# jeffpeterson/hypermerge

Measured on AMD Instinct MI355X. Metric: merged changes/sec (1M docs×8 actors) at 1/2/4/8 GPUs + % HBM roofline, higher is better.
Workload: dtype u32; 1 GPU; C4: 1000000 docs/GPU x 8 actors x 64 changes/doc, map LWW sets; docs_per_gpu=1000000, changes_per_gpu=64000000, ops_per_gpu=96000538, parallelism=doc-shard1

## Files before the change

### hypermerge_amd/csrc/merge_kernels.hip

```cpp
#include <hip/hip_runtime.h>
#include <stdint.h>
#include "../../include/hypermerge_amd.h"
#include "merge_kernels.h"
#include "wave.h"

#ifndef HM_ABLATE
#define HM_ABLATE 0
#endif
#ifndef HM_STAMPS
#define HM_STAMPS 0
#endif
#define HM_NSTAMP 20
#ifndef HM_WAVES_PER_EU_OPL4
#define HM_WAVES_PER_EU_OPL4 3
#endif
#ifndef HM_WAVES_PER_EU_LIST3
#define HM_WAVES_PER_EU_LIST3 3
#endif
#ifndef HM_PRIO_PUSH
#define HM_PRIO_PUSH 2
#endif
#ifndef HM_PRIO_IO
#define HM_PRIO_IO 1
#endif
// ... 6 lines not shown
#ifndef HM_PRIO_K2
#define HM_PRIO_K2 2
#endif
#ifndef HM_PRIO_K1
#define HM_PRIO_K1 3
#endif
#ifndef HM_ASYNC_MAX_OPL
#define HM_ASYNC_MAX_OPL 2
#endif
#ifndef HM_ASYNC_STORES
#define HM_ASYNC_STORES 10
#endif
#ifndef HM_ASYNC_CHECK
#define HM_ASYNC_CHECK 0
#endif
#ifndef HM_WAVES_PER_EU
#define HM_WAVES_PER_EU 5
#endif
#ifndef HM_WAVES_PER_EU_WIDE
#define HM_WAVES_PER_EU_WIDE 4
#endif
#define WAVE 64
#define NA_MAX 8
#define NDEP_MAX 1024
typedef unsigned long long u64;
#if defined(__HIP_DEVICE_COMPILE__)
#define LDS __attribute__((address_space(3)))
#else
#define LDS
#endif

namespace hm {

__device__ __forceinline__ u64 readlane64(u64 v, int l) {
    const uint32_t lo = __builtin_amdgcn_readlane((int)(uint32_t)v, l);
    const uint32_t hi = __builtin_amdgcn_readlane((int)(uint32_t)(v >> 32), l);
    return ((u64)hi << 32) | lo;
}
__device__ __forceinline__ uint32_t shfl32(uint32_t v, int src) {
    return (uint32_t)__builtin_amdgcn_ds_bpermute(src << 2, (int)v);
}
__device__ __forceinline__ u64 shfl64(u64 v, int src) {
    return ((u64)shfl32((uint32_t)(v >> 32), src) << 32) | shfl32((uint32_t)v, src);
}
__device__ __forceinline__ u64 wave_or64(u64 v) {
    for (int o = 1; o < WAVE; o <<= 1) v |= shfl64(v, (int)(threadIdx.x ^ o));
    return v;
}
__device__ __forceinline__ uint32_t wave_excl_scan(uint32_t v, uint32_t *total) {
    uint32_t x = v;
    x += (uint32_t)__builtin_amdgcn_update_dpp(0, (int)x, DPP_ROW_SHR(1), 0xF, 0xF, false);
    x += (uint32_t)__builtin_amdgcn_update_dpp(0, (int)x, DPP_ROW_SHR(2), 0xF, 0xF, false);
    x += (uint32_t)__builtin_amdgcn_update_dpp(0, (int)x, DPP_ROW_SHR(4), 0xF, 0xF, false);
    x += (uint32_t)__builtin_amdgcn_update_dpp(0, (int)x, DPP_ROW_SHR(8), 0xF, 0xF, false);
    x += (uint32_t)__builtin_amdgcn_update_dpp(0, (int)x, DPP_ROW_BCAST15, 0xA, 0xF, false);
    x += (uint32_t)__builtin_amdgcn_update_dpp(0, (int)x, DPP_ROW_BCAST31, 0xC, 0xF, false);
    *total = (uint32_t)__builtin_amdgcn_readlane((int)x, WAVE - 1);
    return x - v;
}
__device__ __forceinline__ uint32_t wave_max(uint32_t v) {
    uint32_t x = v, y;
    y = (uint32_t)__builtin_amdgcn_update_dpp(0, (int)x, DPP_ROW_SHR(1), 0xF, 0xF, false); x = x > y ? x : y;
    y = (uint32_t)__builtin_amdgcn_update_dpp(0, (int)x, DPP_ROW_SHR(2), 0xF, 0xF, false); x = x > y ? x : y;
    y = (uint32_t)__builtin_amdgcn_update_dpp(0, (int)x, DPP_ROW_SHR(4), 0xF, 0xF, false); x = x > y ? x : y;
    y = (uint32_t)__builtin_amdgcn_update_dpp(0, (int)x, DPP_ROW_SHR(8), 0xF, 0xF, false); x = x > y ? x : y;
    y = (uint32_t)__builtin_amdgcn_update_dpp(0, (int)x, DPP_ROW_BCAST15, 0xA, 0xF, false); x = x > y ? x : y;
    y = (uint32_t)__builtin_amdgcn_update_dpp(0, (int)x, DPP_ROW_BCAST31, 0xC, 0xF, false); x = x > y ? x : y;
    return (uint32_t)__builtin_amdgcn_readlane((int)x, WAVE - 1);
}
__device__ __forceinline__ uint32_t bytesum64(u64 x) {
    return __builtin_amdgcn_sad_u8((uint32_t)x, 0u, __builtin_amdgcn_sad_u8((uint32_t)(x >> 32), 0u, 0u));
}
__device__ __forceinline__ uint32_t prev_lane(uint32_t v) {
    return (uint32_t)__builtin_amdgcn_update_dpp(0, (int)v, DPP_WAVE_SHR1, 0xF, 0xF, false);
}
__device__ __forceinline__ uint32_t fresh_lane() {
    uint32_t l;
    asm volatile("v_mov_b32 %0, %1" : "=v"(l) : "v"((uint32_t)threadIdx.x));
    return l;
}
template <bool FRESH> __device__ __forceinline__ uint32_t lane_id() {
    if constexpr (FRESH) return fresh_lane();
    else return threadIdx.x;
}
template <int OPL, bool LISTS, int CLS> struct Diet { static constexpr bool on = OPL <= 2 && !LISTS && CLS != 1; };
__device__ __forceinline__ void wave_sync() {
    __builtin_amdgcn_fence(__ATOMIC_SEQ_CST, "wavefront");
    __builtin_amdgcn_wave_barrier();
}

__device__ __forceinline__ u64 err_key(uint32_t h, uint32_t op_plus1, uint32_t arr, uint32_t code) {
    return ((u64)h << 40) | ((u64)(op_plus1 & 0xFFFF) << 24) | ((u64)(arr & 0xFFFF) << 8) | code;
}

struct SmallLds {
    LDS u64 *anc, *chain, *segor, *errkey, *cov;
    LDS u64 *opval;
    LDS u64 *survpk;
    LDS int64_t *survsum;
    LDS uint32_t *first, *base, *bclock, *headv, *objslot, *segcnt, *survcnt, *regoff, *regobj, *insmin;
    LDS uint32_t *flags, *deps, *depinfo;
    LDS uint8_t *seglist;
    LDS uint16_t *survp;
    LDS uint32_t *opro;
    LDS uint32_t *opmeta;
    LDS uint32_t *opelem;
    LDS int32_t *hist_of;
    LDS uint16_t *survop, *opbase;
    LDS uint16_t *oppar;
    LDS uint8_t *h2a, *chactor, *objtype;
    LDS uint16_t *opchg;
    LDS uint32_t *nins, *pcount, *nodekey, *tour0, *listbase;
    LDS uint16_t *poff;
    LDS uint16_t *nodeop, *nodepi, *regnode, *plist, *fc, *ns, *listid;
    LDS u64 *stamps;
};
#define PAR_HEAD 0xFFFFu
template <bool LISTS> struct Stride {
    static constexpr uint32_t reg = LISTS ? 1 : 4;
    static constexpr uint32_t seg = LISTS ? 1 : 2;
    static constexpr uint32_t op = LISTS ? 1 : 2;
};

template <int CLS> struct SizeClass;
template <> struct SizeClass<0> { static constexpr uint32_t NR = 32, NO = 16, ND = 128; };
template <> struct SizeClass<1> { static constexpr uint32_t NR = 256, NO = 64, ND = 512; };
template <> struct SizeClass<2> { static constexpr uint32_t NR = 128, NO = 32, ND = 256; };

template <typename L_t, typename P>
__host__ __device__ inline size_t small_carve(P base, uint32_t NOp, uint32_t NR, uint32_t NO, uint32_t ND,
                                              bool lists, bool counters, L_t *L) {
    size_t o = 0;
#define TAKE(f, T, cnt) do { L->f = (decltype(L->f))(base + o); o = (o + (size_t)(cnt) * sizeof(T) + 15) & ~(size_t)15; } while (0)
    TAKE(anc, u64, 64);          TAKE(chain, u64, NA_MAX);     TAKE(opval, u64, NOp);
    TAKE(errkey, u64, 1);        TAKE(base, uint32_t, NA_MAX * 3);
    if (lists) {
        TAKE(survcnt, uint32_t, NR); TAKE(regoff, uint32_t, NR);   TAKE(regobj, uint32_t, NR);
        TAKE(insmin, uint32_t, NR);  TAKE(flags, uint32_t, 2);
        TAKE(opmeta, uint32_t, NOp); TAKE(opro, uint32_t, NOp);
    } else {
        TAKE(survcnt, uint32_t, 4 * NR);                           TAKE(flags, uint32_t, 2);
        L->regoff = L->survcnt + 1; L->insmin = L->survcnt + 2;    L->regobj = L->survcnt + 3;
        TAKE(opro, uint32_t, 2 * NOp);
        L->opmeta = L->opro + 1;
    }
    TAKE(survop, uint16_t, NOp); TAKE(chactor, uint8_t, 64);   TAKE(objtype, uint8_t, NO);
    if (lists) {
        TAKE(opelem, uint32_t, NOp);
        L->nodekey = L->opelem;
        TAKE(nins, uint32_t, 1);
    }
    TAKE(stamps, u64, HM_STAMPS ? HM_NSTAMP + 1 : 0);
    const size_t dead_at = o;
    TAKE(hist_of, int32_t, 64);  TAKE(cov, u64, 1);            TAKE(opbase, uint16_t, 64);
    TAKE(oppar, uint16_t, lists ? NOp : 0);
    TAKE(h2a, uint8_t, 64);      TAKE(opchg, uint16_t, NOp);
    const size_t k1_at = o;
    TAKE(first, uint32_t, NA_MAX * 64);
    TAKE(deps, uint32_t, ND > NOp ? ND : NOp);
    TAKE(depinfo, uint32_t, ND);
    const size_t k1_end = o;
    o = k1_at;
    if (lists) { TAKE(segor, u64, NR);  TAKE(survpk, u64, NR); }
    else { TAKE(segor, u64, 2 * NR);    L->survpk = L->segor + 1; }
    TAKE(segcnt, uint32_t, NR);
    TAKE(objslot, uint32_t, NO);
    if (o < k1_end) o = k1_end;
    L->seglist = (decltype(L->seglist))L->first; L->survp = (decltype(L->survp))L->first;
    if (lists) {
        const uint32_t NP = NR + NO, NE = 2 * (NOp + NO);
        size_t q = dead_at;
#define TAKEK(f, T, cnt) do { L->f = (decltype(L->f))(base + q); q = (q + (size_t)(cnt) * sizeof(T) + 15) & ~(size_t)15; } while (0)
        TAKEK(tour0, uint32_t, NE);     TAKEK(pcount, uint32_t, NP);  TAKEK(listbase, uint32_t, NO + 1);
        TAKEK(poff, uint16_t, NP + 1);  TAKEK(survp, uint16_t, NOp);
        TAKEK(nodeop, uint16_t, NOp);   TAKEK(nodepi, uint16_t, NOp); TAKEK(regnode, uint16_t, NR);
        TAKEK(plist, uint16_t, NOp);    TAKEK(fc, uint16_t, NP);      TAKEK(ns, uint16_t, NOp);
        TAKEK(listid, uint16_t, NO);    TAKEK(seglist, uint8_t, NOp);
#undef TAKEK
        if (q > o) o = q;
    }
    TAKE(survsum, int64_t, counters ? NOp : 0);
#undef TAKE
    L->bclock = L->base + NA_MAX;
    L->headv = L->base + 2 * NA_MAX;
    return o;
}

template <typename T> struct Id { typedef T type; };
template <typename T> __device__ __forceinline__ T lds_or(LDS T *p, typename Id<T>::type v) { return __atomic_fetch_or(p, v, __ATOMIC_RELAXED); }
template <typename T> __device__ __forceinline__ T lds_min(LDS T *p, typename Id<T>::type v) { return __atomic_fetch_min(p, v, __ATOMIC_RELAXED); }
template <typename T> __device__ __forceinline__ T lds_max(LDS T *p, typename Id<T>::type v) { return __atomic_fetch_max(p, v, __ATOMIC_RELAXED); }
template <typename T> __device__ __forceinline__ T lds_add(LDS T *p, typename Id<T>::type v) { return __atomic_fetch_add(p, v, __ATOMIC_RELAXED); }

#if HM_STAMPS
__device__ unsigned long long hm_stamp_acc[HM_NSTAMP];
__device__ __forceinline__ u64 stamp_now() {
    u64 t;
    __builtin_amdgcn_sched_barrier(0);
    asm volatile("s_memtime %0\n\ts_waitcnt lgkmcnt(0)" : "=s"(t) :: "memory");
    __builtin_amdgcn_sched_barrier(0);
    return t;
}
#define STAMP(L_, i) do { const u64 t_ = stamp_now(); if (threadIdx.x == 0) { (L_).stamps[i] += t_ - (L_).stamps[HM_NSTAMP]; (L_).stamps[HM_NSTAMP] = t_; } } while (0)
#elif defined(HM_MARKS)
#define STAMP(L_, i) asm volatile(";HMMARK " #i)
#else
#define STAMP(L_, i) do { } while (0)
#endif

enum : uint32_t { FL_UNSUPPORTED = 1u };
enum Outcome { OUT_OK = 0, OUT_ERROR = 1, OUT_UNSUPPORTED = 2, OUT_INVALID = 3 };

__device__ __forceinline__ void need_set(uint32_t &lo, uint32_t &hi, uint32_t a, uint32_t v) {
    const uint32_t sh = (a & 3) * 8;
    const uint32_t w = a < 4 ? lo : hi;
    const uint32_t cur = (w >> sh) & 0xFF;
    const uint32_t nw = v > cur ? ((w & ~(0xFFu << sh)) | (v << sh)) : w;
    lo = a < 4 ? nw : lo;
    hi = a < 4 ? hi : nw;
}


__device__ __forceinline__ uint32_t fidx(uint32_t a, uint32_t s) { return (s & 63) * NA_MAX + (a & (NA_MAX - 1)); }
__device__ __forceinline__ void clear_first(LDS uint32_t *first, uint32_t lane) {
    static_assert(NA_MAX * 64 == 2 * WAVE * 4, "first-table size");
    LDS uint4 *f4 = (LDS uint4 *)first;
    const uint4 ones = make_uint4(~0u, ~0u, ~0u, ~0u);
    f4[lane] = ones;
    f4[lane + WAVE] = ones;
}

__device__ __forceinline__ uint32_t tie_order(uint32_t pc) { return (pc & 1) ? (0x10000u - pc) : (0x20000u + pc); }


template <int OPL>
__device__ __forceinline__ void rga_order(const SmallLds &L, uint32_t R, uint32_t O,
                                          const uint32_t (&oreg)[OPL], const uint32_t (&oobj)[OPL],
                                          const uint32_t (&opar)[OPL], const uint32_t (&oact)[OPL],
                                          const uint32_t (&oelem)[OPL], const uint32_t (&oarr)[OPL],
// ... 327 lines not shown
        if (lane < n) f(lane);
        if constexpr (CAP > WAVE) { if (lane + WAVE < n) f(lane + WAVE); }
    } else {
        for (uint32_t i = lane; i < n; i += WAVE) f(i);
    }
}
template <int OPL, bool LISTS, bool DIET, typename C>
__device__ __forceinline__ void stage_rows(const SmallParams &p, const SmallLds &L, const hm_doc_row &doc, const Rows &r) {
    const uint32_t lane = lane_id<DIET>(), m = doc.n_ops;
    stage_op<LISTS>(L, lane, m, r.a0, r.b0);
    if (OPL > 1) stage_op<LISTS>(L, lane + WAVE, m, r.a1, r.b1);
    if (OPL > 2) stage_op<LISTS>(L, lane + 2 * WAVE, m, r.a2, r.b2);
    if (OPL > 3) stage_op<LISTS>(L, lane + 3 * WAVE, m, r.a3, r.b3);
    const uint32_t nd = doc.n_deps < C::ND ? doc.n_deps : C::ND;
    if (lane < nd) L.deps[lane] = pack_dep(r.d0);
    if (lane + WAVE < nd) L.deps[lane + WAVE] = pack_dep(r.d1);
    if constexpr (C::ND > 2 * WAVE)
        for (uint32_t i = lane + 2 * WAVE; i < nd; i += WAVE)
            L.deps[i] = pack_dep(*reinterpret_cast<const uint2 *>(p.deps + doc.dep_off + i));
}
__device__ __forceinline__ hm_change_row change_of(uint2 w0, uint2 w1, uint2 w2) {
    hm_change_row c;
    c.actor = (uint16_t)(w0.x & 0xFFFF); c.n_deps = (uint16_t)(w0.x >> 16); c.seq = w0.y;
    c.dep_off = w1.x; c.n_ops = w1.y; c.op_first = w2.x; c.content_id = w2.y;
    return c;
}
struct DocState {
    int32_t hist;
    uint32_t H, total;
    bool doc_lists;
    bool counters;
};

struct OpCheck { uint32_t err; bool surv, has_list, late; };
template <bool LISTS>
__device__ __forceinline__ OpCheck op_check(const SmallLds &L, int32_t ohv, uint32_t act, uint32_t obj, uint32_t reg,
                                            uint32_t par, uint32_t okey, uint32_t R, uint32_t O) {
    const bool asg = ohv >= 0 && act >= HM_INS && act <= HM_INC && reg < R;
    const uint32_t oi = obj < O ? obj : 0u, ri = reg < R ? reg : 0u;
    const uint32_t os = obj < O ? L.objslot[oi] : 0xFFFFFFFFu;
    const uint32_t pi = par < R ? par : 0u;
    uint32_t ot = 0, im = 0, ip = 0;
    if constexpr (LISTS) { ot = L.objtype[oi]; im = L.insmin[ri]; ip = L.insmin[pi]; }
    const u64 so = L.segor[Stride<LISTS>::seg * ri];
    const uint32_t h = ohv < 0 ? 0u : (uint32_t)ohv;
    const bool unknown = asg && (os == 0xFFFFFFFFu || os > okey);
    const bool known = asg && !unknown;
    if constexpr (!LISTS) {
        OpCheck r;
        r.has_list = false; r.late = false;
        r.surv = known && (act == HM_SET || act == HM_LINK) && !((so >> h) & 1);
        r.err = unknown ? (uint32_t)HM_ERR_UNKNOWN_OBJECT : 0u;
        return r;
    }
    const bool is_list = ot == HM_MAKE_LIST || ot == HM_MAKE_TEXT;
    const bool ins = known && act == HM_INS;
    const bool sl = known && (act == HM_SET || act == HM_LINK);
    OpCheck r;
    r.has_list = ins || (known && is_list);
    r.surv = sl && !((so >> h) & 1);
    r.late = ins && par != HM_HEAD && !(ip <= okey);
    uint32_t e = 0;
    if (sl && is_list && !(im <= okey)) e = HM_ERR_MISSING_ELEM;
    if (ins && im != okey + 1) e = HM_ERR_DUPLICATE_ELEM;
    if (unknown) e = HM_ERR_UNKNOWN_OBJECT;
    r.err = e;
    return r;
}

template <int OPL, bool LISTS, bool DIET, typename C>
__device__ __forceinline__ Outcome merge_doc_small(const SmallParams &p, const SmallLds &L, const hm_doc_row &doc,
                                                   const uint2 w0, const uint2 w1, const uint2 w2, DocState &st) {
    uint32_t lane = lane_id<DIET>();
    constexpr uint32_t RS = Stride<LISTS>::reg, SS = Stride<LISTS>::seg, OS = Stride<LISTS>::op;
    const uint32_t n = doc.n_changes, A = doc.n_actors, m = doc.n_ops, R = doc.n_regs, O = doc.n_objs;
    st.hist = -1; st.H = 0; st.total = 0; st.doc_lists = false; st.counters = false;

    if (HM_ABLATE & 8) return OUT_UNSUPPORTED;
    STAMP(L, 0);
    if (HM_PRIO_K1) __builtin_amdgcn_s_setprio(HM_PRIO_K1);
    const bool act = lane < n;
    const hm_change_row c = change_of(w0, w1, w2);
    clear_first(L.first, lane);
    if (lane < NA_MAX) { L.base[lane] = 0xFFFFFFFFu; L.bclock[lane] = 0; L.headv[lane] = 0; L.chain[lane] = 0; }
    if (lane == 0) { *L.errkey = ~0ull; L.flags[0] = 0; L.flags[1] = 0; *L.cov = 0; }
    const uint32_t dep_lo = doc.dep_off, ndep = doc.n_deps;
    wave_sync();
    const uint32_t actor = c.actor, seq = c.seq;
    const uint32_t my_dep0 = c.dep_off - dep_lo;
    const uint32_t op_end = c.op_first + c.n_ops, dep_end = c.dep_off + c.n_deps;
    const uint32_t prev_op = prev_lane(op_end), prev_dep = prev_lane(dep_end);
    bool bad = (n == 0 && (m || ndep)) ||
               (act && (c.op_first != (lane ? prev_op : doc.op_off) || c.dep_off != (lane ? prev_dep : dep_lo) ||
                        (lane == n - 1 && (op_end != doc.op_off + m || dep_end != dep_lo + ndep))));
    const bool rowok = act && !(actor >= A || seq == 0 || c.dep_off < dep_lo || my_dep0 + c.n_deps > ndep);
    bad |= act && !rowok;
    bad |= act && (c.op_first < doc.op_off || c.op_first - doc.op_off + c.n_ops > m);
    const uint32_t a8 = actor & (NA_MAX - 1);
    lds_min(&L.base[a8], rowok ? seq : 0xFFFFFFFFu);
    lds_max(&L.bclock[a8], rowok ? seq : 0u);
    L.chactor[lane] = (uint8_t)actor;
    L.opbase[lane] = (uint16_t)(c.op_first - doc.op_off);
    if (__ballot(bad)) return OUT_UNSUPPORTED;
    wave_sync();
    const uint32_t mybase = act ? L.base[a8] : 0;
    const uint32_t slot = seq - mybase;
    if (__ballot(act && slot >= 64)) return OUT_UNSUPPORTED;
    lds_min(&L.first[fidx(a8, (slot & 63))], act ? lane : 0xFFFFFFFFu);
    {
        const uint32_t o0 = c.op_first - doc.op_off;
        if (act) for (uint32_t j = 0; j < c.n_ops; j++) L.opchg[o0 + j] = (uint16_t)(lane | (a8 << 8));
    }
    wave_sync();

    STAMP(L, 1);
    if constexpr (DIET) lane = fresh_lane();
    if (HM_ABLATE & 16) return OUT_UNSUPPORTED;
    {
        bool bad_dep = false;
        for_rows<C::ND, LISTS>(lane, ndep, [&](uint32_t i) {
            const uint32_t pk = L.deps[i];
            const uint32_t a = pk >> 24, s = pk & 0xFFFFFF;
            bad_dep |= pk == 0xFFFFFFFFu || a >= A;
            const uint32_t ad = a & (NA_MAX - 1);
            const uint32_t b = L.base[ad];
            const bool inwin = b != 0xFFFFFFFFu && s >= b && s - b < 64;
            const uint32_t f = L.first[fidx(ad, ((s - b) & 63))];
            const uint32_t rel = s == 0 ? 0u : (inwin ? s - b + 1 : 0x7Fu);
            L.depinfo[i] = (inwin && f < 64 ? f : 0x7Fu) | (rel << 8) | (ad << 16);
        });
        if (__ballot(bad_dep)) return OUT_UNSUPPORTED;
    }
    const uint32_t first_me = act ? L.first[fidx(actor, slot)] : lane;
    const bool dup = act && first_me != lane;
    const uint32_t cid_first = shfl32(c.content_id, (int)(first_me & 63));
    u64 dmask = 0;
    uint32_t pred_arr = 0xFFu;
    bool ok = true;
    bool own_row = false;
    wave_sync();
    {
        const uint32_t maxd = wave_max(act ? (uint32_t)c.n_deps : 0u);
        for (uint32_t j0 = 0; j0 < maxd; j0 += 2) {
            uint32_t inf[2];
#pragma unroll
            for (int u = 0; u < 2; u++) {
                const bool live = act && j0 + u < c.n_deps;
                inf[u] = L.depinfo[live ? my_dep0 + j0 + u : 0u];
            }
#pragma unroll
            for (int u = 0; u < 2; u++) {
                const bool live = act && j0 + u < c.n_deps;
                const uint32_t a = (inf[u] >> 16) & (NA_MAX - 1), rel = (inf[u] >> 8) & 0x7F, f = inf[u] & 0x7F;
                own_row |= live && a == actor;
                const bool use = live && a != actor && rel != 0;
                ok = ok && !(use && (rel == 0x7F || f >= lane));
                dmask |= (use && rel != 0x7F && f < lane) ? (1ull << f) : 0ull;
            }
        }
        const uint32_t ps = seq - 1;
        const bool hp = act && ps != 0, inb = ps >= mybase;
        const uint32_t f = L.first[fidx(a8, ((ps - mybase) & 63))];
        ok = ok && !(hp && (!inb || f >= lane));
        const bool pv = hp && inb && f < lane;
        dmask |= pv ? (1ull << (f & 63)) : 0ull;
        pred_arr = pv ? f : pred_arr;
        ok = ok && !(dup && cid_first != c.content_id);
    }
    wave_sync();

    STAMP(L, 2);
    if constexpr (DIET) lane = fresh_lane();
    if (HM_ABLATE & 32) return OUT_UNSUPPORTED;
    int32_t hist = -1;
    uint32_t H = 0;
    bool identity = false;
    if (HM_PRIO_K1) __builtin_amdgcn_s_setprio(0);
    const bool queued_doc = __ballot(act && !ok) != 0;
    if (HM_PRIO_HIST && queued_doc) __builtin_amdgcn_s_setprio(HM_PRIO_HIST);
    if (!queued_doc) {
        const u64 appl = __ballot(act && !dup);
        if (act) hist = dup ? -2 : (int32_t)__popcll(appl & ((1ull << lane) - 1));
        H = (uint32_t)__popcll(appl);
        identity = __ballot(dup) == 0;
    } else if (__ballot(dup && cid_first != c.content_id) == 0) {
        u64 dall = 0;
        bool never = false;
        uint32_t pred_any = 0xFFu;
        {
            const uint32_t maxd = wave_max(act ? (uint32_t)c.n_deps : 0u);
            for (uint32_t j = 0; j < maxd; j++) {
                const bool live = act && j < c.n_deps;
                const uint32_t inf = L.depinfo[live ? my_dep0 + j : 0u];
                const uint32_t a = (inf >> 16) & (NA_MAX - 1), rel = (inf >> 8) & 0x7F, f = inf & 0x7F;
                const bool use = live && a != actor && rel != 0;
                never |= use && (rel == 0x7F || f == 0x7F);
                dall |= (use && rel != 0x7F && f != 0x7F) ? (1ull << f) : 0ull;
            }
            const uint32_t ps = seq - 1;
            const bool hp = act && ps != 0, inb = ps >= mybase;
            const uint32_t f = L.first[fidx(a8, ((ps - mybase) & 63))];
            never |= hp && (!inb || f >= 64);
            dall |= (hp && inb && f < 64) ? (1ull << f) : 0ull;
            pred_any = (hp && inb && f < 64) ? f : 0xFFu;
        }
        const u64 dupm = __ballot(dup), nodupm = __ballot(act && !dup);
        const u64 below = (1ull << lane) - 1;
        const uint32_t key = first_me & 63;
        u64 applied = 0, queue = 0;
        bool copy_applied = false;
        bool solved = false;
        {
            LDS uint32_t *tx = (LDS uint32_t *)L.hist_of;
            LDS uint32_t *tm = (LDS uint32_t *)L.anc;
            const uint32_t INF = 0xFFu;
            const bool has_dup = dupm != 0;
            const bool kl = act && !dup;
            uint32_t t = (!kl || never) ? INF : lane;
            const bool regdp = __ballot(act && __popcll(dall) > 4) == 0;
            uint32_t sl0 = lane, sl1 = lane, sl2 = lane, sl3 = lane;
            if (regdp) {
                u64 m = dall;
                sl0 = m ? (uint32_t)__builtin_ctzll(m) : lane; m &= m - 1;
                sl1 = m ? (uint32_t)__builtin_ctzll(m) : lane; m &= m - 1;
                sl2 = m ? (uint32_t)__builtin_ctzll(m) : lane; m &= m - 1;
                sl3 = m ? (uint32_t)__builtin_ctzll(m) : lane;
                for (uint32_t it = 0; it <= n; it++) {
                    const uint32_t x0 = shfl32(t, (int)sl0), x1 = shfl32(t, (int)sl1);
                    const uint32_t x2 = shfl32(t, (int)sl2), x3 = shfl32(t, (int)sl3);
                    uint32_t nt = t;
                    nt = nt > x0 ? nt : x0; nt = nt > x1 ? nt : x1; nt = nt > x2 ? nt : x2; nt = nt > x3 ? nt : x3;
                    nt = (kl && t != INF) ? nt : t;
                    const bool grew = nt != t;
                    t = nt;
                    if (__ballot(grew) == 0) break;
                }
            } else {
                for (uint32_t it = 0; it <= n; it++) {
                    tx[lane] = t;
                    wave_sync();
                    uint32_t nt = t;
                    if (kl && t != INF)
                        for (u64 m = dall; m; m &= m - 1) { const uint32_t x = tx[__builtin_ctzll(m)]; nt = nt > x ? nt : x; }
                    wave_sync();
                    const bool grew = nt != t;
                    t = nt;
                    if (__ballot(grew) == 0) break;
                }
            }
            STAMP(L, 13);
            tx[lane] = t;
            wave_sync();
            const uint32_t tk = act ? tx[key] : INF;
            wave_sync();
            uint32_t w = (!kl || t == INF) ? 0xFFFFFFFFu : ((t << 16) | ((t == lane ? 1u : 2u) << 8) | lane);
            bool conv = false;
            if (regdp) {
                const bool queued_copy = act && tk != INF && tk != key && lane < tk;
                const uint32_t nsl = (uint32_t)__popcll(dall);
                for (uint32_t it = 0; it <= n + 1; it++) {
                    const uint32_t y0 = shfl32(w, (int)sl0), y1 = shfl32(w, (int)sl1);
                    const uint32_t y2 = shfl32(w, (int)sl2), y3 = shfl32(w, (int)sl3);
                    uint32_t pc = 2;
                    auto fold = [&](uint32_t wd, uint32_t k) {
                        const uint32_t v = ((wd >> 8) & 0xFFu) + ((wd & 0xFFu) > lane ? 1u : 0u);
                        pc = (k < nsl && (wd >> 16) == tk && v > pc) ? v : pc;
                    };
                    fold(y0, 0); fold(y1, 1); fold(y2, 2); fold(y3, 3);
                    const uint32_t cand = queued_copy ? ((tk << 16) | ((pc > 0xFEu ? 0xFEu : pc) << 8) | lane) : 0xFFFFFFFFu;
                    uint32_t nw = w;
                    if (has_dup) {
                        tm[lane] = 0xFFFFFFFFu;
                        wave_sync();
                        if (cand != 0xFFFFFFFFu) lds_min(&tm[key], cand);
// ... 112 lines not shown
                if (seq - 1 != 0) { pred_arr = L.first[fidx(actor, (seq - 1 - mybase))]; dmask |= 1ull << pred_arr; }
            }
        }
    } else {
        uint32_t need_lo = 0, need_hi = 0;
        if (act) {
#pragma unroll 1
            for (uint32_t j = 0; j < c.n_deps; j++) {
                const uint32_t inf = L.depinfo[my_dep0 + j];
                const uint32_t a = (inf >> 16) & (NA_MAX - 1), rel = (inf >> 8) & 0x7F;
                need_set(need_lo, need_hi, a, (a != actor && rel != 0) ? rel : 0u);
            }
            const uint32_t ps = seq - 1;
            need_set(need_lo, need_hi, a8, ps != 0 ? (ps >= mybase ? ps - mybase + 1 : 0x7Fu) : 0u);
        }
        clear_first(L.first, lane);
        wave_sync();
        uint32_t crel_lo = 0, crel_hi = 0;
        u64 queued = 0;
        bool stop = false;
        for (uint32_t i = 0; i < n && !stop; i++) {
            queued |= 1ull << i;
            u64 above = 0;
            bool first_pass = true;
            for (;;) {
                bool progress = false;
                for (;;) {
                    const uint32_t x0 = ((crel_lo | 0x80808080u) - need_lo) & 0x80808080u;
                    const uint32_t x1 = ((crel_hi | 0x80808080u) - need_hi) & 0x80808080u;
                    u64 r = __ballot(act && x0 == 0x80808080u && x1 == 0x80808080u) & queued;
                    r &= first_pass ? (1ull << i) : above;
                    if (!r) break;
                    const uint32_t j = (uint32_t)__builtin_ctzll(r);
                    const uint32_t aj = (uint32_t)__builtin_amdgcn_readlane((int)actor, (int)j);
                    const uint32_t sj = (uint32_t)__builtin_amdgcn_readlane((int)slot, (int)j);
                    const uint32_t sh = (aj & 3) * 8;
                    const uint32_t cur = (((aj < 4) ? crel_lo : crel_hi) >> sh) & 0xFF;
                    queued &= ~(1ull << j);
                    progress = true;
                    above = (j >= 63) ? 0 : (~0ull << (j + 1));
                    if (sj + 1 <= cur) {
                        const uint32_t k = L.first[fidx(aj, sj)];
                        const uint32_t ck = (uint32_t)__builtin_amdgcn_readlane((int)c.content_id, (int)k);
                        const uint32_t cj = (uint32_t)__builtin_amdgcn_readlane((int)c.content_id, (int)j);
                        if (lane == j) hist = -2;
                        if (ck != cj) {
                            if (lane == 0) lds_min(L.errkey, err_key(H, 0, j, HM_ERR_INCONSISTENT_SEQ));
                            stop = true;
                            break;
                        }
                        if (first_pass) break;
                        continue;
                    }
                    if (aj < 4) crel_lo = (crel_lo & ~(0xFFu << sh)) | ((sj + 1) << sh);
                    else        crel_hi = (crel_hi & ~(0xFFu << sh)) | ((sj + 1) << sh);
                    if (lane == 0) L.first[fidx(aj, sj)] = j;
                    if (lane == j) hist = (int32_t)H;
                    H++;
                    if (first_pass) break;
                }
                if (stop || !progress) break;
                first_pass = false;
                above = ~0ull;
            }
        }
        wave_sync();
        dmask = 0; pred_arr = 0xFFu;
        if (act && hist >= 0) {
            for (uint32_t j = 0; j < c.n_deps; j++) {
                const uint32_t pk = L.deps[my_dep0 + j];
                const uint32_t a = pk >> 24, s = pk & 0xFFFFFF;
                if (a == actor || s == 0) continue;
                dmask |= 1ull << L.first[fidx(a, (s - L.base[a]))];
            }
            if (seq - 1 != 0) { pred_arr = L.first[fidx(actor, (seq - 1 - mybase))]; dmask |= 1ull << pred_arr; }
        }
    }

    if (HM_PRIO_HIST && queued_doc) __builtin_amdgcn_s_setprio(0);
    STAMP(L, 3);
    if constexpr (DIET) lane = fresh_lane();
    if (HM_ABLATE & 512) return OUT_UNSUPPORTED;
    if (act) L.hist_of[lane] = hist;
    if (act && hist >= 0) L.h2a[hist] = (uint8_t)lane;
    wave_sync();
    const bool hv = lane < H;
    uint32_t ai = lane, hactor = actor, hseq = seq, hpred = pred_arr;
    u64 dm_arr = dmask;
    if (!identity) {
        ai = hv ? L.h2a[lane] : 0;
        dm_arr = shfl64(dmask, (int)ai);
        hactor = shfl32(actor, (int)ai); hseq = shfl32(seq, (int)ai); hpred = shfl32(pred_arr, (int)ai);
    }
    u64 D = 0, Dnp = 0;
    if (identity) {
        D = hv ? dm_arr : 0ull;
        Dnp = hv && hpred != 0xFFu ? D & ~(1ull << hpred) : D;
    } else if (hv) {
        u64 x = dm_arr;
        while (x) {
            const uint32_t j = (uint32_t)__builtin_ctzll(x);
            x &= x - 1;
            const u64 bit = 1ull << (uint32_t)L.hist_of[j];
            D |= bit;
            if (j != hpred) Dnp |= bit;
        }
    }
    if (hv) { lds_or(L.cov, D); lds_or(&L.chain[hactor], 1ull << lane); }
    uint32_t alo = hv && lane < 32 ? 1u << lane : 0u, ahi = hv && lane >= 32 ? 1u << (lane - 32) : 0u;
    if (HM_ABLATE & 1024) return OUT_UNSUPPORTED;
    {
        if (HM_PRIO_PUSH) __builtin_amdgcn_s_setprio(HM_PRIO_PUSH);
        const uint32_t Hs = (uint32_t)__builtin_amdgcn_readfirstlane((int)H);
        const uint32_t Dlo = (uint32_t)D, Dhi = (uint32_t)(D >> 32);
        const uint32_t H1 = Hs < 32 ? Hs : 32;
#define PUSH_BC(v, k) ((uint32_t)__builtin_amdgcn_readlane((int)(v), (int)(k)))
#define PUSH_LO(k) alo |= PUSH_BC(alo, (k)) & (uint32_t)__builtin_amdgcn_sbfe((int)Dlo, (k), 1)
#define PUSH_HI(k) do { const uint32_t m_ = (uint32_t)__builtin_amdgcn_sbfe((int)Dhi, (k) - 32, 1);          \
                        const uint32_t bl_ = PUSH_BC(alo, (k)), bh_ = PUSH_BC(ahi, (k));                   \
                        alo |= bl_ & m_; ahi |= bh_ & m_; } while (0)
#pragma unroll
        for (int g = 0; g < 32; g += 8) {
            if ((uint32_t)g >= H1) break;
            PUSH_LO(g); PUSH_LO(g + 1); PUSH_LO(g + 2); PUSH_LO(g + 3);
            PUSH_LO(g + 4); PUSH_LO(g + 5); PUSH_LO(g + 6); PUSH_LO(g + 7);
        }
#pragma unroll
        for (int g = 32; g < 64; g += 8) {
            if ((uint32_t)g >= Hs) break;
            PUSH_HI(g); PUSH_HI(g + 1); PUSH_HI(g + 2); PUSH_HI(g + 3);
            PUSH_HI(g + 4); PUSH_HI(g + 5); PUSH_HI(g + 6); PUSH_HI(g + 7);
        }
#undef PUSH_LO
#undef PUSH_HI
#undef PUSH_BC
        if (HM_PRIO_PUSH) __builtin_amdgcn_s_setprio(0);
    }
    const u64 anc = hv ? ((((u64)ahi << 32) | alo) & ~(1ull << lane)) : 0ull;
    if (hv) L.anc[lane] = anc;
    wave_sync();
    STAMP(L, 4);
    if constexpr (DIET) lane = fresh_lane();
    if (HM_ABLATE & 64) return OUT_UNSUPPORTED;
    const u64 covered = *L.cov;
    bool suspect = false;
    if constexpr (LISTS) {
        if (hv && (Dnp & (Dnp - 1))) {
            u64 x = Dnp;
            while (x) {
                const uint32_t i2 = (uint32_t)__builtin_ctzll(x);
                x &= x - 1;
                if (L.anc[i2] & Dnp) suspect = true;
            }
        }
    } else {
        const u64 rest = Dnp & (Dnp - 1);
        const bool two = hv && rest != 0;
        if (__ballot(two)) {
            const u64 a1 = L.anc[two ? (uint32_t)__builtin_ctzll(rest) : 0u];
            u64 x = two ? rest & (rest - 1) : 0ull;
            suspect = two && (a1 & Dnp) != 0;
            if (__ballot(x != 0)) {
                while (x) {
                    const uint32_t i2 = (uint32_t)__builtin_ctzll(x);
                    x &= x - 1;
                    if (L.anc[i2] & Dnp) suspect = true;
                }
            }
        }
    }
    uint32_t h_own_row = own_row ? 1u : 0u, h_dep0 = my_dep0, h_nd = c.n_deps;
    if (!identity) {
        h_own_row = shfl32(h_own_row, (int)ai); h_dep0 = shfl32(my_dep0, (int)ai); h_nd = shfl32(c.n_deps, (int)ai);
    }
    suspect |= hv && h_own_row != 0;
    if (suspect) {
        const FoldView fv = {L.anc, L.chain, L.first, L.base, L.deps, L.hist_of};
        if (fold_differs(fv, h_dep0, h_nd, hactor, hseq)) lds_or(L.flags, FL_UNSUPPORTED);
    }
    if (hv && !((covered >> lane) & 1)) L.headv[hactor] = hseq;
    for_rows<C::NO, LISTS>(lane, O, [&](uint32_t i) {
        L.objslot[i] = i == 0 ? 0u : 0xFFFFFFFFu;
        if constexpr (LISTS) L.objtype[i] = i == 0 ? HM_MAKE_MAP : 0xFF;
    });
    for_rows<C::NR, LISTS>(lane, R, [&](uint32_t i) {
        if constexpr (LISTS) {
            L.segor[i] = 0; L.segcnt[i] = 0; L.survpk[i] = 0; L.insmin[i] = 0xFFFFFFFFu; L.regobj[i] = HM_NONE;
        } else {
            static_assert(Stride<false>::reg == 4 && Stride<false>::seg == 2, "row widths");
            *(LDS uint4 *)(L.survcnt + 4 * i) = make_uint4(0u, 0u, 0xFFFFFFFFu, HM_NONE);
            *(LDS uint4 *)(L.segor + 2 * i) = make_uint4(0u, 0u, 0u, 0u);
            L.segcnt[i] = 0;
        }
    });
    wave_sync();

    STAMP(L, 5);
    if constexpr (DIET) lane = fresh_lane();
    if (HM_PRIO_K2) __builtin_amdgcn_s_setprio(HM_PRIO_K2);
    if (HM_ABLATE & 2) return OUT_UNSUPPORTED;
    uint32_t oreg[OPL], oobj[OPL], opar[OPL], oact[OPL], okey[OPL], oarr[OPL], oelem[OPL], oactor[OPL];
    int32_t oh[OPL];
    bool counter_ops = false, malformed = false;
    if constexpr (!LISTS) {
        uint2 ow[OPL];
        uint32_t cw[OPL], ob[OPL];
        int32_t hr[OPL];
        u64 an[OPL];
#pragma unroll
        for (int t = 0; t < OPL; t++) { ow[t] = *(LDS uint2 *)(L.opro + 2 * (lane + WAVE * t)); cw[t] = L.opchg[lane + WAVE * t]; }
#pragma unroll
        for (int t = 0; t < OPL; t++) {
            const uint32_t ch = lane + WAVE * t < m ? cw[t] & 0xFFu : 0u;
            oarr[t] = ch; oactor[t] = (cw[t] >> 8) & (NA_MAX - 1);
            ob[t] = L.opbase[ch];
            hr[t] = identity ? (int32_t)ch : L.hist_of[ch];
        }
#pragma unroll
        for (int t = 0; t < OPL; t++) {
            oh[t] = lane + WAVE * t < m ? hr[t] : -1;
            an[t] = L.anc[oh[t] < 0 ? 0 : oh[t]];
        }
        bool listy = false;
#pragma unroll
        for (int t = 0; t < OPL; t++) {
            const uint32_t k = lane + WAVE * t;
            const bool live = k < m, applied = oh[t] >= 0;
            const uint32_t a = live ? ow[t].y & 0xFF : 0xFFu;
            oact[t] = a; oreg[t] = ow[t].x & 0xFFFFu; oobj[t] = ow[t].x >> 16; opar[t] = 0; oelem[t] = 0;
            okey[t] = ((uint32_t)(applied ? oh[t] : 0) << 16) | (k - ob[t]);
            counter_ops |= live & ((a == HM_INC) | (((ow[t].y >> 8) & 0xFF) == HM_DT_COUNTER));
            const bool make = a <= HM_MAKE_TEXT;
            const bool bad = live & (make ? oobj[t] >= O : ((a > HM_INC) | (oreg[t] >= R)));
            malformed |= bad;
            listy |= (a == HM_INS) | (applied & ((a == HM_MAKE_LIST) | (a == HM_MAKE_TEXT)));
            const bool asg = applied & !bad & !make & (a != HM_INS) & (oobj[t] < O);
            if (applied & !bad & make) lds_min(&L.objslot[oobj[t]], okey[t] + 1);
            if (asg) { L.regobj[4 * oreg[t]] = oobj[t]; lds_add(&L.segcnt[oreg[t]], 1u); }
            if (asg && a != HM_INC) lds_or(&L.segor[2 * oreg[t]], an[t]);
        }
        malformed |= listy;
    } else {
#pragma unroll
    for (int t = 0; t < OPL; t++) {
        const uint32_t k = lane + WAVE * t;
        oh[t] = -1; okey[t] = 0; oarr[t] = 0; oreg[t] = 0; oobj[t] = 0; opar[t] = 0; oact[t] = 0xFF; oelem[t] = 0; oactor[t] = 0;
        if (k < m) {
            const uint32_t meta = L.opmeta[k], ro = L.opro[k], pr = L.oppar[k];
            const uint32_t cw = L.opchg[k], ch = cw & 0xFFu;
            oarr[t] = ch; oactor[t] = cw >> 8; oh[t] = identity ? (int32_t)ch : L.hist_of[ch];
            oreg[t] = ro & 0xFFFFu; oobj[t] = ro >> 16; oact[t] = meta & 0xFF;
            opar[t] = pr == PAR_HEAD ? HM_HEAD : pr;
            if (LISTS) {
                oelem[t] = L.opelem[k];
                if (oact[t] == HM_INS && oelem[t] >= (1u << 24)) lds_or(L.flags, FL_UNSUPPORTED);
            }
            counter_ops |= oact[t] == HM_INC || ((meta >> 8) & 0xFF) == HM_DT_COUNTER;
            okey[t] = ((uint32_t)(oh[t] < 0 ? 0 : oh[t]) << 16) | (k - L.opbase[ch]);
            const uint32_t a = oact[t];
            const bool bad = a <= HM_MAKE_TEXT ? oobj[t] >= O
                           : (a <= HM_INC ? (oreg[t] >= R || (a == HM_INS && opar[t] != HM_HEAD && opar[t] >= R)) : true);
            malformed |= bad;
            if (oh[t] >= 0 && !bad) {
                if (a <= HM_MAKE_TEXT) lds_min(&L.objslot[oobj[t]], okey[t] + 1);
                else if (oobj[t] < O) {
                    L.regobj[oreg[t]] = oobj[t];
                    if (a == HM_INS) lds_min(&L.insmin[oreg[t]], okey[t] + 1);
                    else {
                        lds_add(&L.segcnt[oreg[t]], 1u);
                        if (a != HM_INC) lds_or(&L.segor[oreg[t]], L.anc[oh[t]]);
                    }
                }
            }
        }
    }
    }
    STAMP(L, 6);
    if constexpr (DIET) lane = fresh_lane();
    if (HM_ABLATE & 128) return OUT_UNSUPPORTED;
    if (__ballot(malformed)) return OUT_UNSUPPORTED;
    bool doc_counters = false;
    if constexpr (LISTS) {
        if (!p.counters && __ballot(counter_ops)) lds_or(L.flags, FL_UNSUPPORTED);
    } else if (__ballot(counter_ops)) {
        if (p.counters) doc_counters = true;
        else lds_or(L.flags, FL_UNSUPPORTED);
    }
    wave_sync();
#pragma unroll
    for (int t = 0; t < OPL; t++)
        if (oh[t] >= 0 && oact[t] <= HM_MAKE_TEXT && oobj[t] < O) {
            if (L.objslot[oobj[t]] != okey[t] + 1)
                lds_min(L.errkey, err_key((uint32_t)oh[t], (okey[t] & 0xFFFF) + 1, oarr[t], HM_ERR_DUPLICATE_OBJECT));
            else if constexpr (LISTS) L.objtype[oobj[t]] = (uint8_t)oact[t];
        }
    wave_sync();
    bool surv[OPL];
    bool has_list = false, anyerr = false, late = false;
#pragma unroll
    for (int t = 0; t < OPL; t++) {
        const OpCheck ck = op_check<LISTS>(L, oh[t], oact[t], oobj[t], oreg[t], opar[t], okey[t], R, O);
        has_list |= ck.has_list;
        anyerr |= ck.err != 0;
        late |= ck.late;
        surv[t] = ck.surv;
        if (surv[t]) lds_add(&L.survpk[SS * oreg[t]], 1ull << (8 * oactor[t]));
    }
    if (LISTS && __ballot(late)) return OUT_UNSUPPORTED;
    if (__ballot(anyerr)) {
        u64 errk = ~0ull;
#pragma unroll
        for (int t = 0; t < OPL; t++) {
            const OpCheck ck = op_check<LISTS>(L, oh[t], oact[t], oobj[t], oreg[t], opar[t], okey[t], R, O);
            const uint32_t h = oh[t] < 0 ? 0u : (uint32_t)oh[t], kk = (okey[t] & 0xFFFF) + 1;
            const u64 ek = ck.err ? err_key(h, kk, oarr[t], ck.err) : ~0ull;
            errk = errk < ek ? errk : ek;
        }
        lds_min(L.errkey, errk);
    }
    const bool doc_lists = LISTS && __ballot(has_list) != 0;
    wave_sync();
    if (*L.errkey != ~0ull) return OUT_ERROR;
    if (*L.flags & FL_UNSUPPORTED) return OUT_UNSUPPORTED;

    STAMP(L, 7);
    if constexpr (DIET) lane = fresh_lane();
    if (HM_PRIO_K2 && !HM_PRIO_RANK) __builtin_amdgcn_s_setprio(0);
    if (HM_PRIO_RANK) __builtin_amdgcn_s_setprio(HM_PRIO_RANK);
    if (HM_ABLATE & 4) return OUT_UNSUPPORTED;
    uint32_t total = 0;
    const uint32_t lane_s = LISTS ? lane : fresh_lane();
    auto offsets = [&](uint32_t r) {
        uint32_t tot;
        const uint32_t cnt = r < R ? bytesum64(L.survpk[SS * r]) : 0u;
        const uint32_t ex = wave_excl_scan(cnt, &tot);
        if constexpr (LISTS) { if (r < R) { L.regoff[r] = total + ex; L.survcnt[r] = cnt; } }
        else if (r < R) *(LDS uint2 *)(L.survcnt + 4 * r) = make_uint2(cnt, total + ex);
        total += tot;
    };
    if constexpr (C::NR <= 2 * WAVE && !LISTS) {
        offsets(lane_s);
        if constexpr (C::NR > WAVE) { if (R > WAVE) offsets(lane_s + WAVE); }
    } else {
        for (uint32_t r0 = 0; r0 < R; r0 += WAVE) offsets(r0 + lane_s);
    }
    wave_sync();
    uint32_t my_act[OPL], rb0[OPL], rank[OPL];
    bool tie[OPL];
#pragma unroll
    for (int t = 0; t < OPL; t++) {
        const uint32_t ri = surv[t] ? oreg[t] : 0u;
        my_act[t] = surv[t] ? oactor[t] : 0u;
        rb0[t] = L.regoff[RS * ri];
        const u64 pk = L.survpk[SS * ri];
        const uint32_t sh = 8 * (my_act[t] + 1);
        rank[t] = surv[t] ? bytesum64(sh >= 64 ? 0ull : pk >> sh) : 0u;
        tie[t] = surv[t] && ((pk >> (8 * my_act[t])) & 0xFF) > 1;
    }
    bool anytie = false;
#pragma unroll
    for (int t = 0; t < OPL; t++) anytie |= tie[t];
    if (__ballot(anytie)) {
        uint32_t myt[OPL];
        bool oddn[OPL];
#pragma unroll
        for (int t = 0; t < OPL; t++) {
            myt[t] = 0;
            oddn[t] = tie[t] && (L.segcnt[tie[t] ? oreg[t] : 0u] & 1);
            u64 tm = __ballot(tie[t]);
            while (tm) {
                const int j = (int)__builtin_ctzll(tm);
                tm &= tm - 1;
                const uint32_t rj = (uint32_t)__builtin_amdgcn_readlane((int)oreg[t], j);
                const uint32_t kj = (uint32_t)__builtin_amdgcn_readlane((int)okey[t], j);
                uint32_t pc = 0;
#pragma unroll
                for (int t2 = 0; t2 < OPL; t2++)
                    pc += (uint32_t)__popcll(__ballot(oh[t2] >= 0 && oact[t2] >= HM_SET && oact[t2] <= HM_INC &&
                                                      oreg[t2] == rj && okey[t2] < kj));
                if ((int)lane == j) myt[t] = tie_order(pc);
            }
        }
#pragma unroll
        for (int t = 0; t < OPL; t++) {
            u64 tm = __ballot(tie[t]);
            while (tm) {
                const int j = (int)__builtin_ctzll(tm);
                tm &= tm - 1;
                const uint32_t rj = (uint32_t)__builtin_amdgcn_readlane((int)oreg[t], j);
                const uint32_t aj = (uint32_t)__builtin_amdgcn_readlane((int)my_act[t], j);
                const uint32_t tj = (uint32_t)__builtin_amdgcn_readlane((int)myt[t], j);
#pragma unroll
                for (int t2 = 0; t2 < OPL; t2++) {
                    const bool peer = tie[t2] && oreg[t2] == rj && my_act[t2] == aj && !(t2 == t && (int)lane == j);
                    rank[t2] += (peer && (oddn[t2] ? (tj > myt[t2]) : (tj < myt[t2]))) ? 1u : 0u;
                }
            }
        }
    }
#pragma unroll
    for (int t = 0; t < OPL; t++) {
        if (!surv[t]) continue;
        const uint32_t pos = rb0[t] + rank[t];
        uint32_t tag = 0;
        if (LISTS ? p.counters != 0 : doc_counters) {
            const uint32_t mt = L.opmeta[OS * (lane + WAVE * t)], vt = (mt >> 16) & 0xFF;
            const bool cset = (mt & 0xFF) == HM_SET && ((mt >> 8) & 0xFF) == HM_DT_COUNTER && (vt == HM_V_INT || vt == HM_V_FLOAT);
            tag = cset ? (0x8000u | (vt == HM_V_INT ? 0x4000u : 0u) | ((uint32_t)oh[t] << 8)) : 0u;
            L.survsum[pos] = 0;
        }
        L.survop[pos] = (uint16_t)((lane + WAVE * t) | tag);
    }
    wave_sync();
    if (HM_PRIO_RANK) __builtin_amdgcn_s_setprio(0);
    STAMP(L, 8);
    if constexpr (DIET) lane = fresh_lane();
    if (HM_ABLATE & 256) return OUT_UNSUPPORTED;
    if constexpr (LISTS) {
        if (doc_lists)
            rga_order<OPL>(L, R, O, oreg, oobj, opar, oact, oelem, oarr, oh, p.res_epos ? p.res_epos + doc.reg_off : nullptr);
    }
    if (LISTS ? (p.counters && __ballot(counter_ops)) : doc_counters) {
        bool outside = false;
        int64_t incv[OPL];
        u64 basev[OPL];
#pragma unroll
        for (int t = 0; t < OPL; t++) {
            incv[t] = (oh[t] >= 0 && oact[t] == HM_INC) ? (int64_t)op_value(L, lane + WAVE * t) : 0;
            const uint32_t q = lane + WAVE * t;
            basev[t] = 0;
            if (q < total) {
                const uint32_t sw = L.survop[q];
                if ((sw & 0xC000u) == 0xC000u) basev[t] = op_value(L, sw & 0xFFu);
            }
        }
#pragma unroll
        for (int t = 0; t < OPL; t++) {
            if (oh[t] < 0 || oact[t] != HM_INC) continue;
            const uint32_t k = lane + WAVE * t;
            const uint32_t reg = oreg[t], b0 = L.regoff[RS * reg], cnt = L.survcnt[RS * reg];
            const u64 an = L.anc[oh[t]];
            const uint32_t my_vtag = (L.opmeta[OS * k] >> 16) & 0xFF;
            const int64_t v = incv[t];
            for (uint32_t q = 0; q < cnt; q++) {
                const uint32_t sw = L.survop[b0 + q];
// ... 379 lines not shown
```

Measured before the change: 34.64 billion changes/s.

## Trim DIET merge path: opaque ballots, named-dep flags, unrolled opchg writes

```diff
diff --git a/hypermerge_amd/csrc/merge_kernels.hip b/hypermerge_amd/csrc/merge_kernels.hip
--- a/hypermerge_amd/csrc/merge_kernels.hip
+++ b/hypermerge_amd/csrc/merge_kernels.hip
@@ -112,6 +112,11 @@
 template <bool FRESH> __device__ __forceinline__ uint32_t lane_id() {
     if constexpr (FRESH) return fresh_lane();
     else return threadIdx.x;
+}
+template <bool OPAQUE> __device__ __forceinline__ bool wave_any(bool x) {
+    u64 b = __ballot(x);
+    if constexpr (OPAQUE) asm("" : "+s"(b));
+    return b != 0;
 }
 template <int OPL, bool LISTS, int CLS> struct Diet { static constexpr bool on = OPL <= 2 && !LISTS && CLS != 1; };
 __device__ __forceinline__ void wave_sync() {
@@ -139,6 +144,7 @@
     LDS uint16_t *survop, *opbase;
     LDS uint16_t *oppar;
     LDS uint8_t *h2a, *chactor, *objtype;
+    LDS uint8_t *named;
     LDS uint16_t *opchg;
     LDS uint32_t *nins, *pcount, *nodekey, *tour0, *listbase;
     LDS uint16_t *poff;
@@ -185,6 +191,7 @@
     TAKE(hist_of, int32_t, 64);  TAKE(cov, u64, 1);            TAKE(opbase, uint16_t, 64);
     TAKE(oppar, uint16_t, lists ? NOp : 0);
     TAKE(h2a, uint8_t, 64);      TAKE(opchg, uint16_t, NOp);
+    L->named = L->h2a;
     const size_t k1_at = o;
     TAKE(first, uint32_t, NA_MAX * 64);
     TAKE(deps, uint32_t, ND > NOp ? ND : NOp);
@@ -678,7 +685,10 @@
     const bool act = lane < n;
     const hm_change_row c = change_of(w0, w1, w2);
     clear_first(L.first, lane);
-    if (lane < NA_MAX) { L.base[lane] = 0xFFFFFFFFu; L.bclock[lane] = 0; L.headv[lane] = 0; L.chain[lane] = 0; }
+    if (lane < NA_MAX) {
+        L.base[lane] = 0xFFFFFFFFu; L.bclock[lane] = 0; L.headv[lane] = 0; L.chain[lane] = 0;
+        if constexpr (DIET) ((LDS u64 *)L.named)[lane] = 0;
+    }
     if (lane == 0) { *L.errkey = ~0ull; L.flags[0] = 0; L.flags[1] = 0; *L.cov = 0; }
     const uint32_t dep_lo = doc.dep_off, ndep = doc.n_deps;
     wave_sync();
@@ -697,15 +707,23 @@
     lds_max(&L.bclock[a8], rowok ? seq : 0u);
     L.chactor[lane] = (uint8_t)actor;
     L.opbase[lane] = (uint16_t)(c.op_first - doc.op_off);
-    if (__ballot(bad)) return OUT_UNSUPPORTED;
+    if (wave_any<DIET>(bad)) return OUT_UNSUPPORTED;
     wave_sync();
     const uint32_t mybase = act ? L.base[a8] : 0;
     const uint32_t slot = seq - mybase;
-    if (__ballot(act && slot >= 64)) return OUT_UNSUPPORTED;
+    if (wave_any<DIET>((DIET || act) && slot >= 64)) return OUT_UNSUPPORTED;
     lds_min(&L.first[fidx(a8, (slot & 63))], act ? lane : 0xFFFFFFFFu);
     {
         const uint32_t o0 = c.op_first - doc.op_off;
-        if (act) for (uint32_t j = 0; j < c.n_ops; j++) L.opchg[o0 + j] = (uint16_t)(lane | (a8 << 8));
+        const uint16_t cw = (uint16_t)(lane | (a8 << 8));
+        if constexpr (DIET) {
+            if (!wave_any<DIET>(c.n_ops > 2)) {
+                if (act && c.n_ops > 0) L.opchg[o0] = cw;
+                if (act && c.n_ops > 1) L.opchg[o0 + 1] = cw;
+            } else if (act) {
+                for (uint32_t j = 0; j < c.n_ops; j++) { L.opchg[o0 + j] = cw; asm volatile(""); }
+            }
+        } else if (act) for (uint32_t j = 0; j < c.n_ops; j++) L.opchg[o0 + j] = cw;
     }
     wave_sync();
 
@@ -725,7 +743,7 @@
             const uint32_t rel = s == 0 ? 0u : (inwin ? s - b + 1 : 0x7Fu);
             L.depinfo[i] = (inwin && f < 64 ? f : 0x7Fu) | (rel << 8) | (ad << 16);
         });
-        if (__ballot(bad_dep)) return OUT_UNSUPPORTED;
+        if (wave_any<DIET>(bad_dep)) return OUT_UNSUPPORTED;
     }
     const uint32_t first_me = act ? L.first[fidx(actor, slot)] : lane;
     const bool dup = act && first_me != lane;
@@ -736,8 +754,8 @@
     bool own_row = false;
     wave_sync();
     {
-        const uint32_t maxd = wave_max(act ? (uint32_t)c.n_deps : 0u);
-        for (uint32_t j0 = 0; j0 < maxd; j0 += 2) {
+        const uint32_t maxd = DIET ? 0u : wave_max(act ? (uint32_t)c.n_deps : 0u);
+        for (uint32_t j0 = 0; DIET ? wave_any<DIET>(j0 < c.n_deps) : j0 < maxd; j0 += 2) {
             uint32_t inf[2];
 #pragma unroll
             for (int u = 0; u < 2; u++) {
@@ -751,7 +769,9 @@
                 own_row |= live && a == actor;
                 const bool use = live && a != actor && rel != 0;
                 ok = ok && !(use && (rel == 0x7F || f >= lane));
-                dmask |= (use && rel != 0x7F && f < lane) ? (1ull << f) : 0ull;
+                const bool met = use && rel != 0x7F && f < lane;
+                dmask |= met ? (1ull << f) : 0ull;
+                if constexpr (DIET) { if (met) L.named[f] = 1; }
             }
         }
         const uint32_t ps = seq - 1;
@@ -760,6 +780,7 @@
         ok = ok && !(hp && (!inb || f >= lane));
         const bool pv = hp && inb && f < lane;
         dmask |= pv ? (1ull << (f & 63)) : 0ull;
+        if constexpr (DIET) { if (pv) L.named[f & 63] = 1; }
         pred_arr = pv ? f : pred_arr;
         ok = ok && !(dup && cid_first != c.content_id);
     }
@@ -772,20 +793,20 @@
     uint32_t H = 0;
     bool identity = false;
     if (HM_PRIO_K1) __builtin_amdgcn_s_setprio(0);
-    const bool queued_doc = __ballot(act && !ok) != 0;
+    const bool queued_doc = wave_any<DIET>(act && !ok);
     if (HM_PRIO_HIST && queued_doc) __builtin_amdgcn_s_setprio(HM_PRIO_HIST);
     if (!queued_doc) {
         const u64 appl = __ballot(act && !dup);
         if (act) hist = dup ? -2 : (int32_t)__popcll(appl & ((1ull << lane) - 1));
         H = (uint32_t)__popcll(appl);
-        identity = __ballot(dup) == 0;
-    } else if (__ballot(dup && cid_first != c.content_id) == 0) {
+        identity = !wave_any<DIET>(dup);
+    } else if (!wave_any<DIET>(dup && cid_first != c.content_id)) {
         u64 dall = 0;
         bool never = false;
         uint32_t pred_any = 0xFFu;
         {
-            const uint32_t maxd = wave_max(act ? (uint32_t)c.n_deps : 0u);
-            for (uint32_t j = 0; j < maxd; j++) {
+            const uint32_t maxd = DIET ? 0u : wave_max(act ? (uint32_t)c.n_deps : 0u);
+            for (uint32_t j = 0; DIET ? wave_any<DIET>(j < c.n_deps) : j < maxd; j++) {
                 const bool live = act && j < c.n_deps;
                 const uint32_t inf = L.depinfo[live ? my_dep0 + j : 0u];
                 const uint32_t a = (inf >> 16) & (NA_MAX - 1), rel = (inf >> 8) & 0x7F, f = inf & 0x7F;
@@ -1064,7 +1085,7 @@
     if constexpr (DIET) lane = fresh_lane();
     if (HM_ABLATE & 512) return OUT_UNSUPPORTED;
     if (act) L.hist_of[lane] = hist;
-    if (act && hist >= 0) L.h2a[hist] = (uint8_t)lane;
+    if ((!DIET || !identity) && act && hist >= 0) L.h2a[hist] = (uint8_t)lane;
     wave_sync();
     const bool hv = lane < H;
     uint32_t ai = lane, hactor = actor, hseq = seq, hpred = pred_arr;
@@ -1088,7 +1109,7 @@
             if (j != hpred) Dnp |= bit;
         }
     }
-    if (hv) { lds_or(L.cov, D); lds_or(&L.chain[hactor], 1ull << lane); }
+    if (hv) { if (!DIET || !identity) lds_or(L.cov, D); lds_or(&L.chain[hactor], 1ull << lane); }
     uint32_t alo = hv && lane < 32 ? 1u << lane : 0u, ahi = hv && lane >= 32 ? 1u << (lane - 32) : 0u;
     if (HM_ABLATE & 1024) return OUT_UNSUPPORTED;
     {
@@ -1138,11 +1159,11 @@
     } else {
         const u64 rest = Dnp & (Dnp - 1);
         const bool two = hv && rest != 0;
-        if (__ballot(two)) {
+        if (wave_any<DIET>(DIET ? rest != 0 : two)) {
             const u64 a1 = L.anc[two ? (uint32_t)__builtin_ctzll(rest) : 0u];
             u64 x = two ? rest & (rest - 1) : 0ull;
             suspect = two && (a1 & Dnp) != 0;
-            if (__ballot(x != 0)) {
+            if (wave_any<DIET>(x != 0)) {
                 while (x) {
                     const uint32_t i2 = (uint32_t)__builtin_ctzll(x);
                     x &= x - 1;
@@ -1160,7 +1181,9 @@
         const FoldView fv = {L.anc, L.chain, L.first, L.base, L.deps, L.hist_of};
         if (fold_differs(fv, h_dep0, h_nd, hactor, hseq)) lds_or(L.flags, FL_UNSUPPORTED);
     }
-    if (hv && !((covered >> lane) & 1)) L.headv[hactor] = hseq;
+    bool listed = ((covered >> lane) & 1) != 0;
+    if constexpr (DIET) { if (identity) listed = L.named[lane] != 0; }
+    if (hv && !listed) L.headv[hactor] = hseq;
     for_rows<C::NO, LISTS>(lane, O, [&](uint32_t i) {
         L.objslot[i] = i == 0 ? 0u : 0xFFFFFFFFu;
         if constexpr (LISTS) L.objtype[i] = i == 0 ? HM_MAKE_MAP : 0xFF;
@@ -1260,11 +1283,11 @@
     STAMP(L, 6);
     if constexpr (DIET) lane = fresh_lane();
     if (HM_ABLATE & 128) return OUT_UNSUPPORTED;
-    if (__ballot(malformed)) return OUT_UNSUPPORTED;
+    if (wave_any<DIET>(malformed)) return OUT_UNSUPPORTED;
     bool doc_counters = false;
     if constexpr (LISTS) {
         if (!p.counters && __ballot(counter_ops)) lds_or(L.flags, FL_UNSUPPORTED);
-    } else if (__ballot(counter_ops)) {
+    } else if (wave_any<DIET>(counter_ops)) {
         if (p.counters) doc_counters = true;
         else lds_or(L.flags, FL_UNSUPPORTED);
     }
@@ -1289,7 +1312,7 @@
         if (surv[t]) lds_add(&L.survpk[SS * oreg[t]], 1ull << (8 * oactor[t]));
     }
     if (LISTS && __ballot(late)) return OUT_UNSUPPORTED;
-    if (__ballot(anyerr)) {
+    if (wave_any<DIET>(anyerr)) {
         u64 errk = ~0ull;
 #pragma unroll
         for (int t = 0; t < OPL; t++) {
@@ -1342,7 +1365,7 @@
     bool anytie = false;
 #pragma unroll
     for (int t = 0; t < OPL; t++) anytie |= tie[t];
-    if (__ballot(anytie)) {
+    if (wave_any<DIET>(anytie)) {
         uint32_t myt[OPL];
         bool oddn[OPL];
 #pragma unroll
```

Measured after the change: 33.68 billion changes/s. 0.972x the previous value.
